# mmwillet/TTS.cpp

Measured on AMD Instinct MI355X. Metric: audio-seconds/sec (Parler-TTS-Mini fp16, greedy decode + DAC to 44.1 kHz PCM), higher is better.
Workload: dtype f16

## Files before the change

tts.cpp_amd/csrc/parler_kernels.h:

```cpp
#pragma once
#include <hip/hip_runtime.h>
#include <stdint.h>
#include <type_traits>

#include "wave_ops.h"

struct EmbedArgs {
    const void *tab;
    int         tab_f16;
    int64_t     tab_stride;
    int         n_tabs;
    const uint32_t *ids;
    const float *pos_embed;
    const uint32_t *row_pos;
    float      *x;
    int         H;
};

static __global__ void embed_rows_kernel(EmbedArgs a) {
    const int r = blockIdx.x;
    const uint32_t pos = a.row_pos[r];
    uint32_t id[16];
#pragma unroll
    for (int i = 0; i < 16; i++) id[i] = a.ids[r * a.n_tabs + min(i, a.n_tabs - 1)];
// ... 445 lines not shown
__global__ void gemv_valu_kernel(GemmArgs a, int EPI, int act_f16_src) {
    const int lane = threadIdx.x & 63, w = threadIdx.x >> 6;
    const int n = blockIdx.x * (blockDim.x >> 6) + w;
    if (n >= a.N) return;
    for (int r = 0; r < a.R; r++) {
        float acc = 0.0f;
        for (int k = lane; k < a.K; k += 64) {
            float wv, xv;
            if (WT == 1) wv = (float) ((const _Float16 *) a.W)[(int64_t) n * a.K + k];
            else         wv = ((const float *) a.W)[(int64_t) n * a.K + k];
            if (act_f16_src) xv = (float) ((const _Float16 *) a.A)[(int64_t) r * a.lda + k];
            else {
                xv = ((const float *) a.A)[(int64_t) r * a.lda + k];
                if (WT == 1) xv = (float) (_Float16) xv;
            }
            acc += wv * xv;
        }
        acc = wave_sum(acc);
        if (lane == 0) {
            if (EPI == EPI_STORE) a.out[(int64_t) r * a.ldo + n] = acc;
            else if (EPI == EPI_RESID) a.out[(int64_t) r * a.ldo + n] += acc;
            else if (EPI == EPI_GELU) {
                const float gl = gelu_apply(acc, a.gelu_mode);
                if (a.out16) a.out16[(int64_t) r * a.ldo + n] = (_Float16) gl;
                else a.out[(int64_t) r * a.ldo + n] = gl;
            } else {
                const int which = n / a.H, c = n - which * a.H;
                if (which == 0) a.q[(int64_t) r * a.H + c] = acc;
                else {
                    const int64_t off = (int64_t) a.row_seq[r] * a.seq_stride + (int64_t) a.row_pos[r] * a.H + c;
                    void *base = which == 1 ? a.kc : a.vc;
                    if (a.kv_f16) ((_Float16 *) base)[off] = (_Float16) acc;
                    else ((float *) base)[off] = acc;
                }
            }
        }
    }
}

__device__ __forceinline__ unsigned quant4_q8(float4v y, float &d_out);
template <int NI, int NP>
__device__ __forceinline__ void ln_row_regs(float *xr, int H, int lane, const float *lw, const float *lb, float *yr32, _Float16 *yr16,
                                            const float *pr, int n_parts, int64_t slab_stride, int8_t *yq = nullptr, float *ydT = nullptr, int ldr = 0) {
    float4v v[NI], w4[NI], b4[NI];
    float4v p[NP > 0 ? NP : 1][NI];
#pragma unroll
    for (int i = 0; i < NI; i++) {
        const int k = min(i * 256 + lane * 4, H - 4);
        v[i] = *(const float4v *) (xr + k);
#pragma unroll
        for (int sp = 0; sp < NP; sp++) p[sp][i] = *(const float4v *) (pr + sp * slab_stride + k);
        w4[i] = *(const float4v *) (lw + k);
        b4[i] = *(const float4v *) (lb + k);
    }
    if (NP != 0) {
#pragma unroll
        for (int i = 0; i < NI; i++) {
            const int k = i * 256 + lane * 4;
            if (k < H) {
                if (NP > 0) {
#pragma unroll
                    for (int sp = 0; sp < NP; sp++) v[i] += p[sp][i];
                } else {
                    for (int sp = 0; sp < n_parts; sp++) v[i] += *(const float4v *) (pr + sp * slab_stride + k);
                }
                *(float4v *) (xr + k) = v[i];
            }
        }
    }
    float s = 0.0f;
#pragma unroll
    for (int i = 0; i < NI; i++)
        if (i * 256 + lane * 4 < H) s += (v[i][0] + v[i][1]) + (v[i][2] + v[i][3]);
    const float mean = wave_sum(s) / (float) H;
    float s2 = 0.0f;
#pragma unroll
    for (int i = 0; i < NI; i++)
        if (i * 256 + lane * 4 < H) {
#pragma unroll
            for (int e = 0; e < 4; e++) { const float d = v[i][e] - mean; s2 += d * d; }
        }
    const float rstd = 1.0f / sqrtf(wave_sum(s2) / (float) H + LN_EPS);
#pragma unroll
    for (int i = 0; i < NI; i++) {
        const int k = i * 256 + lane * 4;
        if (k < H) {
            float4v y;
#pragma unroll
            for (int e = 0; e < 4; e++) y[e] = (v[i][e] - mean) * rstd * w4[i][e] + b4[i][e];
            if (yr32) *(float4v *) (yr32 + k) = y;
            if (yr16) {
                half4 h;
#pragma unroll
                for (int e = 0; e < 4; e++) h[e] = (_Float16) y[e];
                *(half4 *) (yr16 + k) = h;
            }
            if (yq) {
                float dd;
                const unsigned qq = quant4_q8(y, dd);
                *(unsigned *) (yq + k) = qq;
                if ((lane & 7) == 0) ydT[(int64_t) (k >> 5) * ldr] = dd;
            }
        }
    }
}

template <int NI, int NP>
__global__ __launch_bounds__(256) void ln_rows_t_kernel(float *x, int H, const float *lw, const float *lb, float *y32, _Float16 *y16, int R, const float *parts, int n_parts,
                                                        int64_t slab_stride) {
    const int lane = threadIdx.x & 63;
    const int r = blockIdx.x * (blockDim.x >> 6) + (threadIdx.x >> 6);
    if (r >= R) return;
    const float *pr = parts ? parts + (int64_t) r * H : nullptr;
    ln_row_regs<NI, NP>(x + (int64_t) r * H, H, lane, lw, lb, y32 ? y32 + (int64_t) r * H : nullptr, y16 ? y16 + (int64_t) r * H : nullptr, pr, parts ? n_parts : 0, slab_stride);
}

template <int NI, int NP>
__global__ __launch_bounds__(256) void ln_rows_q8t_kernel(float *x, int H, const float *lw, const float *lb, int8_t *q, float *dT, int ldr, int R, const float *parts, int n_parts,
                                                          int64_t slab_stride) {
    const int lane = threadIdx.x & 63;
    const int r = blockIdx.x * (blockDim.x >> 6) + (threadIdx.x >> 6);
    if (r >= R) return;
    const float *pr = parts ? parts + (int64_t) r * H : nullptr;
    ln_row_regs<NI, NP>(x + (int64_t) r * H, H, lane, lw, lb, (float *) nullptr, (_Float16 *) nullptr, pr, parts ? n_parts : 0, slab_stride, q + (int64_t) r * H, dT + r, ldr);
}

static __global__ __launch_bounds__(256) void ln_rows_kernel(float *x, int H, const float *lw, const float *lb, float *y32,
                                                      _Float16 *y16, int R, const float *parts, int n_parts, int64_t slab_stride) {
    const int lane = threadIdx.x & 63;
    const int r = blockIdx.x * (blockDim.x >> 6) + (threadIdx.x >> 6);
    if (r >= R) return;
    float *xr = x + (int64_t) r * H;
    if (parts)
        for (int k = lane; k < H; k += 64) {
            float v = xr[k];
            for (int sp = 0; sp < n_parts; sp++) v += parts[sp * slab_stride + (int64_t) r * H + k];
            xr[k] = v;
        }
    float s = 0.0f;
    for (int k = lane; k < H; k += 64) s += xr[k];
    const float mean = wave_sum(s) / (float) H;
    float s2 = 0.0f;
    for (int k = lane; k < H; k += 64) { const float d = xr[k] - mean; s2 += d * d; }
    const float rstd = 1.0f / sqrtf(wave_sum(s2) / (float) H + LN_EPS);
    for (int k = lane; k < H; k += 64) {
        const float y = (xr[k] - mean) * rstd * lw[k] + lb[k];
        if (y32) y32[(int64_t) r * H + k] = y;
        if (y16) y16[(int64_t) r * H + k] = (_Float16) y;
    }
}

struct AttnArgs {
    const float *q;
    const void *kc, *vc;
    int kv_f16;
    int64_t seq_stride;
    const uint32_t *row_seq, *row_pos;
    int T_fixed;
    int H, n_heads;
    float scale;
    float *out;
    _Float16 *out16;
    float *part;
    int max_T;
    uint32_t *counters;
    long long *stamps;
    int8_t *out_q;
    float *out_dT;
    int ldr;
};

__device__ __forceinline__ float4v load_kv4(const void *base, int kv_f16, int64_t off) {
    if (kv_f16) {
        const half4 h = *(const half4 *) ((const _Float16 *) base + off);
        return (float4v){(float) h[0], (float) h[1], (float) h[2], (float) h[3]};
    }
    return *(const float4v *) ((const float *) base + off);
}

template <bool KVF16>
__device__ __forceinline__ void attn_key_pass(const AttnArgs &a, int64_t hb, float4v q4, int tbeg, int t1, int step, int NKG, float &m, float &l, float4v &acc) {
    for (int t = tbeg; t < t1; t += step) {
        float4v k4[4], v4[4];
#pragma unroll
        for (int u = 0; u < 4; u++) {
            const int64_t off = hb + (int64_t) min(t + u * NKG, t1 - 1) * a.H;
            if (KVF16) {
                const half4 hk = *(const half4 *) ((const _Float16 *) a.kc + off), hv = *(const half4 *) ((const _Float16 *) a.vc + off);
                k4[u] = (float4v){(float) hk[0], (float) hk[1], (float) hk[2], (float) hk[3]};
                v4[u] = (float4v){(float) hv[0], (float) hv[1], (float) hv[2], (float) hv[3]};
            } else {
                k4[u] = *(const float4v *) ((const float *) a.kc + off);
                v4[u] = *(const float4v *) ((const float *) a.vc + off);
            }
        }
#pragma unroll
        for (int u = 0; u < 4; u++) {
            if (t + u * NKG < t1) {
                float d = q4[0] * k4[u][0] + q4[1] * k4[u][1] + q4[2] * k4[u][2] + q4[3] * k4[u][3];
                d = row16_sum(d);
                d *= a.scale;
                const float mn = fmaxf(m, d);
                const float f = expf(m - mn);
                const float p = expf(d - mn);
                l = l * f + p;
#pragma unroll
                for (int e = 0; e < 4; e++) acc[e] = acc[e] * f + p * v4[u][e];
                m = mn;
            }
        }
    }
}

static __global__ __launch_bounds__(1024) void attn_kernel(AttnArgs a) {
    extern __shared__ __attribute__((aligned(16))) char smem[];
    const int NKG = blockDim.x >> 4;
    float *red = (float *) smem;
    const int h = blockIdx.x, r = blockIdx.y, z = blockIdx.z, nz = gridDim.z;
    const int tid = threadIdx.x, kg = tid >> 4, cl = tid & 15, c4 = cl * 4;
    B1_STAMP(a.stamps, 0);
    const int T = a.row_pos ? (int) a.row_pos[r] + 1 : a.T_fixed;
    const int64_t sb = a.row_seq ? (int64_t) a.row_seq[r] * a.seq_stride : 0;
    const int chunk = (T + nz - 1) / nz;
    const int t0 = z * chunk, t1 = min(T, t0 + chunk);
    const int64_t hb = sb + h * 64 + c4;
    const float4v q4 = *(const float4v *) (a.q + (int64_t) r * a.H + h * 64 + c4);
    const int step = NKG * 4;

    float m = -INFINITY, l = 0.0f;
    float4v acc = {0.f, 0.f, 0.f, 0.f};
    if (a.kv_f16) attn_key_pass<true>(a, hb, q4, t0 + kg, t1, step, NKG, m, l, acc);
    else attn_key_pass<false>(a, hb, q4, t0 + kg, t1, step, NKG, m, l, acc);
    if (a.stamps != nullptr) { asm volatile("" :: "v"(acc[0])); B1_STAMP(a.stamps, 1); }
    if (cl == 0) red[NKG * 64 + kg] = m;
    __syncthreads();
    float mx = -INFINITY;
    for (int i = 0; i < NKG; i++) mx = fmaxf(mx, red[NKG * 64 + i]);
    const float f = (m == -INFINITY) ? 0.0f : expf(m - mx);
#pragma unroll
    for (int e = 0; e < 4; e++) acc[e] *= f;
    *(float4v *) (red + kg * 64 + c4) = acc;
    if (cl == 0) red[NKG * 65 + kg] = l * f;
    __syncthreads();
    if (tid < 64) {
        float o = 0.0f, s = 0.0f;
        for (int i = 0; i < NKG; i++) { o += red[i * 64 + tid]; s += red[NKG * 65 + i]; }
        if (nz == 1) {
            const float res = o / s;
            if (a.out16) a.out16[(int64_t) r * a.H + h * 64 + tid] = (_Float16) res;
            else a.out[(int64_t) r * a.H + h * 64 + tid] = res;
        } else {
            float *p = a.part + (((int64_t) r * a.n_heads + h) * nz + z) * ATT_PS;
            if (a.counters) {
                if (tid == 0) {
                    __hip_atomic_store(p, mx, __ATOMIC_RELAXED, __HIP_MEMORY_SCOPE_AGENT);
                    __hip_atomic_store(p + 1, s, __ATOMIC_RELAXED, __HIP_MEMORY_SCOPE_AGENT);
                }
                __hip_atomic_store(p + ATT_PO + tid, o, __ATOMIC_RELAXED, __HIP_MEMORY_SCOPE_AGENT);
            } else {
                if (tid == 0) { p[0] = mx; p[1] = s; }
                p[ATT_PO + tid] = o;
            }
        }
    }
    B1_STAMP(a.stamps, 2);
    if (nz == 1 || !a.counters) return;
    uint32_t *s_last = (uint32_t *) (red + NKG * 66);
    __syncthreads();
    if (tid == 0) {
        const uint32_t prev = __hip_atomic_fetch_add(a.counters + r * a.n_heads + h, 1u, __ATOMIC_ACQ_REL, __HIP_MEMORY_SCOPE_AGENT);
        *s_last = prev == (uint32_t) nz - 1 ? 1u : 0u;
    }
    __syncthreads();
    if (!*s_last || tid >= 64) return;
    const float *p = a.part + ((int64_t) r * a.n_heads + h) * nz * ATT_PS;
    float mm[16], ss[16], oo[16];
#pragma unroll
    for (int i = 0; i < 16; i++) {
        if (i < nz) {
            mm[i] = __hip_atomic_load(p + i * ATT_PS, __ATOMIC_RELAXED, __HIP_MEMORY_SCOPE_AGENT);
            ss[i] = __hip_atomic_load(p + i * ATT_PS + 1, __ATOMIC_RELAXED, __HIP_MEMORY_SCOPE_AGENT);
            oo[i] = __hip_atomic_load(p + i * ATT_PS + ATT_PO + tid, __ATOMIC_RELAXED, __HIP_MEMORY_SCOPE_AGENT);
        }
    }
    float gmx = -INFINITY;
#pragma unroll
    for (int i = 0; i < 16; i++) if (i < nz) gmx = fmaxf(gmx, mm[i]);
    float ot = 0.0f, st = 0.0f;
#pragma unroll
    for (int i = 0; i < 16; i++) {
        if (i < nz && mm[i] != -INFINITY) {
            const float f2 = expf(mm[i] - gmx);
            ot += f2 * oo[i];
            st += f2 * ss[i];
        }
    }
    const float res = ot / st;
    if (a.out16) a.out16[(int64_t) r * a.H + h * 64 + tid] = (_Float16) res;
    else a.out[(int64_t) r * a.H + h * 64 + tid] = res;
    if (tid == 0) __hip_atomic_store(a.counters + r * a.n_heads + h, 0u, __ATOMIC_RELAXED, __HIP_MEMORY_SCOPE_AGENT);
    if (a.stamps != nullptr && tid == 0 && (h == 0 || h == (int) gridDim.x - 1) && r == 0) a.stamps[(h ? 8 : 0) + 3] = (long long) __builtin_amdgcn_s_memrealtime();
}

template <bool KVF16, int U>
__device__ __forceinline__ void attn_row_pass(const AttnArgs &a, int64_t hb, float4v q4, int t0, int t1, float &m, float &l, float4v &acc) {
    for (int t = t0; t < t1; t += U) {
        float4v k4[U], v4[U];
#pragma unroll
        for (int u = 0; u < U; u++) {
            const int64_t off = hb + (int64_t) min(t + u, t1 - 1) * a.H;
            if (KVF16) {
                const half4 hk = __builtin_nontemporal_load((const half4 *) ((const _Float16 *) a.kc + off)), hv = __builtin_nontemporal_load((const half4 *) ((const _Float16 *) a.vc + off));
                k4[u] = (float4v){(float) hk[0], (float) hk[1], (float) hk[2], (float) hk[3]};
                v4[u] = (float4v){(float) hv[0], (float) hv[1], (float) hv[2], (float) hv[3]};
            } else {
                k4[u] = __builtin_nontemporal_load((const float4v *) ((const float *) a.kc + off));
                v4[u] = __builtin_nontemporal_load((const float4v *) ((const float *) a.vc + off));
            }
        }
#pragma unroll
        for (int u = 0; u < U; u++) {
            if (t + u < t1) {
                float d = q4[0] * k4[u][0] + q4[1] * k4[u][1] + q4[2] * k4[u][2] + q4[3] * k4[u][3];
                d = row16_sum(d);
                d *= a.scale;
                const float mn = fmaxf(m, d);
                const float f = expf(m - mn);
                const float p = expf(d - mn);
                l = l * f + p;
#pragma unroll
                for (int e = 0; e < 4; e++) acc[e] = acc[e] * f + p * v4[u][e];
                m = mn;
            }
        }
    }
}
template <int U>
__global__ __launch_bounds__(1024) void attn_rows_kernel(AttnArgs a) {
    const int r = blockIdx.x, z = blockIdx.y, nz = gridDim.y, tid = threadIdx.x;
    const int h = tid >> 4, cl = tid & 15;
    const int T = (int) a.row_pos[r] + 1;
    const int64_t sb = (int64_t) a.row_seq[r] * a.seq_stride;
    const int chunk = (T + nz - 1) / nz;
    const int t0 = z * chunk, t1 = min(T, t0 + chunk);
    const int64_t hb = sb + tid * 4;
    const float4v q4 = *(const float4v *) (a.q + (int64_t) r * a.H + tid * 4);
    float m = -INFINITY, l = 0.0f;
    float4v acc = {0.f, 0.f, 0.f, 0.f};
    if (t0 < t1) {
        if (a.kv_f16) attn_row_pass<true, U>(a, hb, q4, t0, t1, m, l, acc);
        else attn_row_pass<false, U>(a, hb, q4, t0, t1, m, l, acc);
    }
    if (nz == 1) {
        const float inv = 1.0f / l;
        if (a.out16) {
            half4 o;
#pragma unroll
            for (int e = 0; e < 4; e++) o[e] = (_Float16) (acc[e] * inv);
            *(half4 *) (a.out16 + (int64_t) r * a.H + tid * 4) = o;
        } else {
            float4v o;
#pragma unroll
            for (int e = 0; e < 4; e++) o[e] = acc[e] * inv;
            if (a.out_q) {
                float dd;
                const unsigned qq = quant4_q8(o, dd);
                *(unsigned *) (a.out_q + (int64_t) r * a.H + tid * 4) = qq;
                if ((tid & 7) == 0) a.out_dT[(int64_t) (tid >> 3) * a.ldr + r] = dd;
            } else {
                *(float4v *) (a.out + (int64_t) r * a.H + tid * 4) = o;
            }
        }
    } else {
        float *p = a.part + (((int64_t) r * a.n_heads + h) * nz + z) * ATT_PS;
        if (cl == 0) { p[0] = m; p[1] = l; }
        *(float4v *) (p + ATT_PO + cl * 4) = acc;
    }
}

template <int TN>
__device__ __forceinline__ void attn_short_body(const AttnArgs &a, int r, int h, int lane, int T) {
    const int64_t hb = h * 64 + lane;
    const float qv = a.q[(int64_t) r * a.H + hb];
    float kv[TN], vv[TN], sc[TN];
    const float *kc = (const float *) a.kc, *vc = (const float *) a.vc;
#pragma unroll
    for (int t = 0; t < TN; t++) {
        const int64_t off = hb + (int64_t) min(t, T - 1) * a.H;
        kv[t] = kc[off];
        vv[t] = vc[off];
    }
    float m = -INFINITY;
#pragma unroll
    for (int t = 0; t < TN; t++)
        if (t < T) { sc[t] = wave_sum(qv * kv[t]) * a.scale; m = fmaxf(m, sc[t]); }
    float l = 0.0f, o = 0.0f;
#pragma unroll
    for (int t = 0; t < TN; t++)
        if (t < T) { const float p = expf(sc[t] - m); l += p; o += p * vv[t]; }
    const float res = o / l;
    if (a.out16) a.out16[(int64_t) r * a.H + hb] = (_Float16) res;
    else a.out[(int64_t) r * a.H + hb] = res;
}
static __global__ __launch_bounds__(256) void attn_short_kernel(AttnArgs a) {
    const int lane = threadIdx.x & 63;
    const int h = blockIdx.x * (blockDim.x >> 6) + (threadIdx.x >> 6), r = blockIdx.y;
    if (h >= a.n_heads) return;
    B1_STAMP(a.stamps, 0);
    const int T = a.T_fixed;
    if (T <= 8) attn_short_body<8>(a, r, h, lane, T);
    else if (T <= 16) attn_short_body<16>(a, r, h, lane, T);
    else attn_short_body<32>(a, r, h, lane, T);
    B1_STAMP(a.stamps, 3);
}


static __global__ void attn_combine_kernel(const float *part, int nz, int H, int n_heads, float *out, _Float16 *out16, int8_t *out_q = nullptr, float *out_dT = nullptr, int ldr = 0) {
    const int h = blockIdx.x, r = blockIdx.y, c = threadIdx.x;
    const float *p = part + ((int64_t) r * n_heads + h) * nz * ATT_PS;
    float m[16], s[16], o[16];
#pragma unroll
    for (int z = 0; z < 16; z++) {
        if (z < nz) { m[z] = p[z * ATT_PS]; s[z] = p[z * ATT_PS + 1]; o[z] = p[z * ATT_PS + ATT_PO + c]; }
    }
    float mx = -INFINITY;
#pragma unroll
    for (int z = 0; z < 16; z++) if (z < nz) mx = fmaxf(mx, m[z]);
    float oo = 0.0f, ss = 0.0f;
#pragma unroll
    for (int z = 0; z < 16; z++) {
        if (z < nz && m[z] != -INFINITY) {
            const float f = expf(m[z] - mx);
            oo += f * o[z];
            ss += f * s[z];
        }
    }
    const float res = oo / ss;
    if (out_q) {
        const float amax = lanes32_max(fabsf(res));
        const float dd = amax / 127.0f;
        const float id = dd ? 1.0f / dd : 0.0f;
        out_q[(int64_t) r * H + h * 64 + c] = (int8_t) roundf(res * id);
        if ((c & 31) == 0) out_dT[(int64_t) (h * 2 + (c >> 5)) * ldr + r] = (float) (_Float16) dd;
    } else if (out16) out16[(int64_t) r * H + h * 64 + c] = (_Float16) res;
    else out[(int64_t) r * H + h * 64 + c] = res;
}

static __global__ void argmax_kernel(const float *logits, int V, uint32_t *tokens) {
    __shared__ float bv[4];
    __shared__ uint32_t bi[4];
    const int idx = blockIdx.x;
    const float *lg = logits + (int64_t) idx * V;
    float best = -INFINITY;
    uint32_t besti = 0;
    for (int i = threadIdx.x; i < V; i += blockDim.x) {
        const float v = lg[i];
        if (v > best) { best = v; besti = (uint32_t) i; }
    }
#pragma unroll
    for (int o = 32; o > 0; o >>= 1) {
        const float ov = __shfl_xor(best, o);
        const uint32_t oi = __shfl_xor(besti, o);
        if (ov > best || (ov == best && oi < besti)) { best = ov; besti = oi; }
    }
    const int w = threadIdx.x >> 6;
    if ((threadIdx.x & 63) == 0) { bv[w] = best; bi[w] = besti; }
    __syncthreads();
    if (threadIdx.x == 0) {
        for (int i = 1; i < (int) (blockDim.x >> 6); i++)
            if (bv[i] > best || (bv[i] == best && bi[i] < besti)) { best = bv[i]; besti = bi[i]; }
        tokens[idx] = besti;
    }
}

#define SMP_VMAX 2048
struct SampleArgs {
    const float *logits;
    int V, n_out, R;
    uint32_t top_k;
    float top_p, temperature;
    const float *uniforms;
    const uint32_t *row_step;
    uint32_t *out;
    const double *pen_table;
    int pen_len;
    int32_t *last_ids;
    uint32_t *rep_counts;
    const uint32_t *orig;
    int R_total;
};

__device__ __forceinline__ unsigned long long smp_key(float v, int i) {
    unsigned u = __float_as_uint(v == 0.0f ? 0.0f : v);
    u = (u & 0x80000000u) ? ~u : (u | 0x80000000u);
    return ((unsigned long long) (~u) << 32) | (unsigned) i;
}

__device__ __forceinline__ void smp_rank_select(const float *val, int V, int k, unsigned short *picks, unsigned long long *keys) {
    int P = 1;
    while (P < V) P <<= 1;
    for (int i = threadIdx.x; i < P; i += blockDim.x) keys[i] = i < V ? smp_key(val[i], i) : ~0ull;
    __syncthreads();
    for (int size = 2; size <= P; size <<= 1) {
        for (int stride = size >> 1; stride > 0; stride >>= 1) {
            for (int t = threadIdx.x; t < (P >> 1); t += blockDim.x) {
                const int lo = ((t / stride) * (stride << 1)) + (t % stride), hi = lo + stride;
                const bool up = ((lo & size) == 0);
                const unsigned long long a = keys[lo], b = keys[hi];
                if ((a > b) == up) { keys[lo] = b; keys[hi] = a; }
            }
            __syncthreads();
        }
    }
    for (int j = threadIdx.x; j < k; j += blockDim.x) picks[j] = (unsigned short) (keys[j] & 0xFFFFu);
}

static __global__ __launch_bounds__(256) void sample_kernel(SampleArgs a) {
    __shared__ float val[SMP_VMAX];
    __shared__ float tmp[SMP_VMAX];
    __shared__ unsigned short picks[SMP_VMAX];
    __shared__ unsigned long long keys[SMP_VMAX];
    __shared__ float bv[4];
    __shared__ uint32_t bi[4];
    __shared__ float s_top, s_total, s_mhp;
    __shared__ int s_n;
    const int h = blockIdx.x, r = blockIdx.y, tid = threadIdx.x, V = a.V;
    const float *row = a.logits + ((int64_t) r * a.n_out + h) * V;
    const bool temp = a.temperature != 1.0f;
    const bool use_topk = a.top_k > 0 && a.top_k < (uint32_t) V;
    const bool use_topp = a.top_p < 1.0f;

    const int ro = a.orig ? (int) a.orig[r] : r;
    const int last = a.pen_table ? a.last_ids[ro * a.n_out + h] : -1;
    float pen_v = 0.0f;
    if (last >= 0 && last < V) {
        const uint32_t cnt = a.rep_counts[ro * a.n_out + h];
        pen_v = (float) ((double) row[last] / a.pen_table[cnt < (uint32_t) a.pen_len ? cnt : (uint32_t) a.pen_len - 1]);
    }
    float best = -INFINITY;
    uint32_t besti = 0;
    for (int i = tid; i < V; i += 256) {
        const float v = i == last ? pen_v : row[i];
        val[i] = v;
        if (v > best) { best = v; besti = (uint32_t) i; }
    }
#pragma unroll
    for (int o = 32; o > 0; o >>= 1) {
        const float ov = __shfl_xor(best, o);
        const uint32_t oi = __shfl_xor(besti, o);
        if (ov > best || (ov == best && oi < besti)) { best = ov; besti = oi; }
    }
    if ((tid & 63) == 0) { bv[tid >> 6] = best; bi[tid >> 6] = besti; }
    __syncthreads();
    if (tid == 0) {
        for (int i = 1; i < 4; i++)
            if (bv[i] > best || (bv[i] == best && bi[i] < besti)) { best = bv[i]; besti = bi[i]; }
        float top = val[besti];
        if (temp) top /= a.temperature;
        s_top = top;
    }
    __syncthreads();
    const float top = s_top;
    int n = V;
    bool nucleus = false;

    if (use_topp) {
        for (int i = tid; i < V; i += 256) {
            float v = val[i];
            if (temp) v /= a.temperature;
            tmp[i] = expf(v - top);
        }
        __syncthreads();
        if (tid == 0) {
            float total = 0.0f;
            for (int i = 0; i < V; i++) total += tmp[i];
            s_total = total;
        }
        __syncthreads();
        for (int i = tid; i < V; i += 256) val[i] = tmp[i] / s_total;
        __syncthreads();
    }
    if (use_topk) {
        smp_rank_select(val, V, (int) a.top_k, picks, keys);
        n = (int) a.top_k;
        nucleus = true;
        __syncthreads();
    }
    if (!use_topp) {
        for (int j = tid; j < n; j += 256) {
            float v = val[nucleus ? picks[j] : j];
            if (temp) v /= a.temperature;
            tmp[j] = expf(v - top);
        }
        __syncthreads();
        if (tid == 0) {
            float total = 0.0f;
            for (int j = 0; j < n; j++) total += tmp[j];
            s_total = total;
        }
        __syncthreads();
        for (int j = tid; j < n; j += 256) val[nucleus ? picks[j] : j] = tmp[j] / s_total;
        __syncthreads();
    } else {
        if (!nucleus) {
            smp_rank_select(val, V, V, picks, keys);
            nucleus = true;
            __syncthreads();
        }
        if (tid == 0) {
            float mass = 0.0f;
            int keep = -1;
            for (int j = 0; j < n; j++) {
                mass += val[picks[j]];
                if (mass >= a.top_p) { keep = j + 1; break; }
            }
            s_mhp = fminf(mass, a.top_p);
            s_n = keep > 0 ? keep : n;
        }
        __syncthreads();
        n = s_n;
    }
    if (tid == 0) {
        const uint32_t call = a.row_step ? a.row_step[r] - 1 : 0;
        const float u = a.uniforms[((int64_t) call * (a.orig ? a.R_total : a.R) + ro) * a.n_out + h];
        const float target = use_topp ? u * s_mhp : u;
        float cum = 0.0f;
        int chosen = n ? (nucleus ? (int) picks[n - 1] : n - 1) : 0;
        for (int j = 0; j < n; j++) {
            const int i = nucleus ? (int) picks[j] : j;
            cum += val[i];
            if (target <= cum || j + 1 >= n) { chosen = i; break; }
        }
        a.out[r * a.n_out + h] = (uint32_t) chosen;
        if (a.pen_table) {
            uint32_t cnt = a.rep_counts[ro * a.n_out + h];
            if (last != chosen) cnt = 0;
            a.last_ids[ro * a.n_out + h] = chosen;
            a.rep_counts[ro * a.n_out + h] = cnt + 1;
        }
    }
}

struct FeedArgs {
    const uint32_t *tokens;
    uint32_t *ids;
    uint32_t *row_pos;
    uint32_t *row_step;
    uint8_t  *eos_seen;
    uint32_t *steps_done;
    uint32_t *tokens_out;
    int R, n_out;
    uint32_t bos, eos;
    uint32_t max_pos;
    const uint32_t *orig;
// ... 242 lines not shown
```

Before: 1016.

## Double-buffer K/V loads in row attention and pin waves per EU

```diff
diff --git a/profiles/attn_rows_bench.hip b/profiles/attn_rows_bench.hip
--- /dev/null
+++ b/profiles/attn_rows_bench.hip
@@ -0,0 +1,339 @@
+#include <hip/hip_runtime.h>
+#include <cstdio>
+#include <cstdlib>
+#include <cstring>
+#include <cmath>
+#include <vector>
+#include <algorithm>
+#include "../tts.cpp_amd/csrc/parler_kernels.h"
+#define CK(x) do { hipError_t e = (x); if (e != hipSuccess) { printf("HIP error %s line %d\n", hipGetErrorString(e), __LINE__); exit(1); } } while (0)
+
+typedef AttnArgs Args;
+
+__global__ void fill_kernel(float *p, size_t n, uint32_t seed, float amp) {
+    for (size_t i = (size_t) blockIdx.x * blockDim.x + threadIdx.x; i < n; i += (size_t) gridDim.x * blockDim.x) {
+        uint32_t x = (uint32_t) i * 2654435761u ^ (uint32_t) (i >> 32) ^ seed;
+        x ^= x >> 16; x *= 0x7feb352du; x ^= x >> 15; x *= 0x846ca68bu; x ^= x >> 16;
+        p[i] = ((float) (x & 0xffffff) / 8388608.0f - 1.0f) * amp;
+    }
+}
+
+template <bool CLAMP>
+__global__ __launch_bounds__(1024) void probe_kernel(Args a) {
+    const int r = blockIdx.x, tid = threadIdx.x;
+    const int T = (int) a.row_pos[r] + 1;
+    const int64_t hb = (int64_t) a.row_seq[r] * a.seq_stride + tid * 4;
+    float4v acc = {0.f, 0.f, 0.f, 0.f};
+    for (int t = 0; t < T; t += 8) {
+        float4v k4[8], v4[8];
+#pragma unroll
+        for (int u = 0; u < 8; u++) {
+            if (CLAMP || t + u < T) {
+                const int64_t off = hb + (int64_t) min(t + u, T - 1) * a.H;
+                k4[u] = __builtin_nontemporal_load((const float4v *) ((const float *) a.kc + off));
+                v4[u] = __builtin_nontemporal_load((const float4v *) ((const float *) a.vc + off));
+            } else {
+                k4[u] = v4[u] = (float4v){0.f, 0.f, 0.f, 0.f};
+            }
+        }
+#pragma unroll
+        for (int u = 0; u < 8; u++) {
+            typedef int int4v __attribute__((ext_vector_type(4)));
+            const int4v x = __builtin_bit_cast(int4v, k4[u]) ^ __builtin_bit_cast(int4v, v4[u]) ^ __builtin_bit_cast(int4v, acc);
+            acc = __builtin_bit_cast(float4v, x);
+        }
+    }
+    if (__builtin_bit_cast(unsigned, acc[0]) == 0x12345678u && __builtin_bit_cast(unsigned, acc[1]) == 0x9abcdef0u) a.out[tid] = acc[2] + acc[3];
+}
+
+template <bool KVF16, int U>
+__device__ __forceinline__ void parent_row_pass(const AttnArgs &a, int64_t hb, float4v q4, int t0, int t1, float &m, float &l, float4v &acc) {
+    for (int t = t0; t < t1; t += U) {
+        float4v k4[U], v4[U];
+#pragma unroll
+        for (int u = 0; u < U; u++) {
+            const int64_t off = hb + (int64_t) min(t + u, t1 - 1) * a.H;
+            if (KVF16) {
+                const half4 hk = __builtin_nontemporal_load((const half4 *) ((const _Float16 *) a.kc + off)), hv = __builtin_nontemporal_load((const half4 *) ((const _Float16 *) a.vc + off));
+                k4[u] = (float4v){(float) hk[0], (float) hk[1], (float) hk[2], (float) hk[3]};
+                v4[u] = (float4v){(float) hv[0], (float) hv[1], (float) hv[2], (float) hv[3]};
+            } else {
+                k4[u] = __builtin_nontemporal_load((const float4v *) ((const float *) a.kc + off));
+                v4[u] = __builtin_nontemporal_load((const float4v *) ((const float *) a.vc + off));
+            }
+        }
+#pragma unroll
+        for (int u = 0; u < U; u++) {
+            if (t + u < t1) {
+                float d = q4[0] * k4[u][0] + q4[1] * k4[u][1] + q4[2] * k4[u][2] + q4[3] * k4[u][3];
+                d = row16_sum(d);
+                d *= a.scale;
+                const float mn = fmaxf(m, d);
+                const float f = expf(m - mn);
+                const float p = expf(d - mn);
+                l = l * f + p;
+#pragma unroll
+                for (int e = 0; e < 4; e++) acc[e] = acc[e] * f + p * v4[u][e];
+                m = mn;
+            }
+        }
+    }
+}
+template <int U>
+__global__ __launch_bounds__(1024) void parent_rows_kernel(AttnArgs a) {
+    const int r = blockIdx.x, z = blockIdx.y, nz = gridDim.y, tid = threadIdx.x;
+    const int h = tid >> 4, cl = tid & 15;
+    const int T = (int) a.row_pos[r] + 1;
+    const int64_t sb = (int64_t) a.row_seq[r] * a.seq_stride;
+    const int chunk = (T + nz - 1) / nz;
+    const int t0 = z * chunk, t1 = min(T, t0 + chunk);
+    const int64_t hb = sb + tid * 4;
+    const float4v q4 = *(const float4v *) (a.q + (int64_t) r * a.H + tid * 4);
+    float m = -INFINITY, l = 0.0f;
+    float4v acc = {0.f, 0.f, 0.f, 0.f};
+    if (t0 < t1) {
+        if (a.kv_f16) parent_row_pass<true, U>(a, hb, q4, t0, t1, m, l, acc);
+        else parent_row_pass<false, U>(a, hb, q4, t0, t1, m, l, acc);
+    }
+    if (nz == 1) {
+        const float inv = 1.0f / l;
+        if (a.out16) {
+            half4 o;
+#pragma unroll
+            for (int e = 0; e < 4; e++) o[e] = (_Float16) (acc[e] * inv);
+            *(half4 *) (a.out16 + (int64_t) r * a.H + tid * 4) = o;
+        } else {
+            float4v o;
+#pragma unroll
+            for (int e = 0; e < 4; e++) o[e] = acc[e] * inv;
+            if (a.out_q) {
+                float dd;
+                const unsigned qq = quant4_q8(o, dd);
+                *(unsigned *) (a.out_q + (int64_t) r * a.H + tid * 4) = qq;
+                if ((tid & 7) == 0) a.out_dT[(int64_t) (tid >> 3) * a.ldr + r] = dd;
+            } else {
+                *(float4v *) (a.out + (int64_t) r * a.H + tid * 4) = o;
+            }
+        }
+    } else {
+        float *p = a.part + (((int64_t) r * a.n_heads + h) * nz + z) * ATT_PS;
+        if (cl == 0) { p[0] = m; p[1] = l; }
+        *(float4v *) (p + ATT_PO + cl * 4) = acc;
+    }
+}
+
+template <int U> using KV = AttnGroup<false, U>;
+template <int U>
+__device__ __forceinline__ void issue(KV<U> &b, const float *rk, const float *rv, int H, int t, int tl, unsigned lo) {
+    attn_issue_group<false, U>(b, (const char *) rk, (const char *) rv, (int64_t) H * 4, t, tl, lo);
+}
+template <int U, bool SKIPF>
+__device__ __forceinline__ void fold(const KV<U> &b, float4v q4, float scale, int t, int t1, float &m, float &l, float4v &acc) {
+    if (!SKIPF) { attn_fold_group<false, U, false>(b, q4, scale, t, t1, m, l, acc); return; }
+#pragma unroll
+    for (int u = 0; u < U; u++) {
+        if (t + u < t1) {
+#pragma clang fp contract(off)
+            const float4v k = b.k[u], v = b.v[u];
+            float d = q4[0] * k[0] + q4[1] * k[1];
+            d = q4[2] * k[2] + d;
+            d = q4[3] * k[3] + d;
+            d = row16_sum(d);
+            const float mn = fmaxf(m, d * scale);
+            const float p = expf(__builtin_fmaf(scale, d, -mn));
+            float f = 1.0f;
+            if (__builtin_amdgcn_ballot_w64(mn != m) != 0) f = mn == m ? 1.0f : expf(m - mn);
+            l = __builtin_fmaf(l, f, p);
+            acc[0] = __builtin_fmaf(v[0], p, acc[0] * f);
+            acc[1] = __builtin_fmaf(v[1], p, acc[1] * f);
+            acc[2] = v[2] * p + acc[2] * f;
+            acc[3] = v[3] * p + acc[3] * f;
+            m = mn;
+        }
+    }
+}
+
+template <int U, bool PIPE, int THREADS, int MINB, bool PERSIST, bool SKIPF>
+__global__ __launch_bounds__(THREADS, MINB) __attribute__((amdgpu_waves_per_eu(THREADS * MINB / 256, THREADS * MINB / 256))) void var_kernel(Args a) {
+    const int tid = threadIdx.x;
+    const unsigned lo = (unsigned) (blockIdx.y * THREADS + tid) * 16u;
+    const int G = gridDim.x;
+    int r = blockIdx.x;
+    if (!PERSIST) {
+        const int T = (int) a.row_pos[r] + 1;
+        const int64_t sb = (int64_t) a.row_seq[r] * a.seq_stride;
+        const float *rk = (const float *) a.kc + sb, *rv = (const float *) a.vc + sb;
+        const float4v q4 = *(const float4v *) ((const char *) (a.q + (int64_t) r * a.H) + lo);
+        float m = -INFINITY, l = 0.0f;
+        float4v acc = {0.f, 0.f, 0.f, 0.f};
+        if (PIPE) {
+            KV<U> A, B;
+            issue<U>(A, rk, rv, a.H, 0, T - 1, lo);
+            for (int t = 0; t < T; t += 2 * U) {
+                issue<U>(B, rk, rv, a.H, t + U, T - 1, lo);
+                fold<U, SKIPF>(A, q4, a.scale, t, T, m, l, acc);
+                if (t + U >= T) break;
+                issue<U>(A, rk, rv, a.H, t + 2 * U, T - 1, lo);
+                fold<U, SKIPF>(B, q4, a.scale, t + U, T, m, l, acc);
+            }
+        } else {
+            for (int t = 0; t < T; t += U) {
+                KV<U> A;
+                issue<U>(A, rk, rv, a.H, t, T - 1, lo);
+                fold<U, SKIPF>(A, q4, a.scale, t, T, m, l, acc);
+            }
+        }
+        const float inv = 1.0f / l;
+        float4v o;
+#pragma unroll
+        for (int e = 0; e < 4; e++) o[e] = acc[e] * inv;
+        *(float4v *) ((char *) (a.out + (int64_t) r * a.H) + lo) = o;
+    } else {
+        int pr = r, pt = 0, pT = (int) a.row_pos[r] + 1;
+        int64_t psb = (int64_t) a.row_seq[r] * a.seq_stride;
+        float4v pq = *(const float4v *) ((const char *) (a.q + (int64_t) r * a.H) + lo);
+        int cr = r, ct = 0, cT = pT;
+        float4v q4 = pq;
+        float m = -INFINITY, l = 0.0f;
+        float4v acc = {0.f, 0.f, 0.f, 0.f};
+        KV<U> A, B;
+        issue<U>(A, (const float *) a.kc + psb, (const float *) a.vc + psb, a.H, 0, pT - 1, lo);
+#define ADVANCE_AND_ISSUE(BUF) \
+        pt += U; \
+        if (pt >= pT && pr + G < a.T_fixed ) { \
+            pr += G; pt = 0; pT = (int) a.row_pos[pr] + 1; psb = (int64_t) a.row_seq[pr] * a.seq_stride; \
+            pq = *(const float4v *) ((const char *) (a.q + (int64_t) pr * a.H) + lo); \
+        } \
+        issue<U>(BUF, (const float *) a.kc + psb, (const float *) a.vc + psb, a.H, pt, pT - 1, lo);
+#define FOLD_AND_STEP(BUF) \
+        fold<U, SKIPF>(BUF, q4, a.scale, ct, cT, m, l, acc); \
+        ct += U; \
+        if (ct >= cT) { \
+            const float inv = 1.0f / l; \
+            float4v o; \
+            for (int e = 0; e < 4; e++) o[e] = acc[e] * inv; \
+            *(float4v *) ((char *) (a.out + (int64_t) cr * a.H) + lo) = o; \
+            cr += G; \
+            if (cr >= a.T_fixed ) break; \
+            ct = 0; cT = pT; q4 = pq; m = -INFINITY; l = 0.0f; acc = (float4v){0.f, 0.f, 0.f, 0.f}; \
+        }
+        for (;;) {
+            ADVANCE_AND_ISSUE(B)
+            FOLD_AND_STEP(A)
+            ADVANCE_AND_ISSUE(A)
+            FOLD_AND_STEP(B)
+        }
+#undef ADVANCE_AND_ISSUE
+#undef FOLD_AND_STEP
+    }
+}
+
+struct Bench {
+    Args a;
+    std::vector<float> h_ref, h_out;
+    size_t n_out;
+    int R;
+    double bytes;
+    int T;
+};
+
+template <typename F>
+static float time_launch(F launch, int reps) {
+    hipEvent_t e0, e1; CK(hipEventCreate(&e0)); CK(hipEventCreate(&e1));
+    launch(); launch();
+    CK(hipDeviceSynchronize());
+    std::vector<float> ms(reps);
+    for (int i = 0; i < reps; i++) {
+        CK(hipEventRecord(e0));
+        launch();
+        CK(hipEventRecord(e1)); CK(hipEventSynchronize(e1));
+        CK(hipEventElapsedTime(&ms[i], e0, e1));
+    }
+    CK(hipGetLastError());
+    std::sort(ms.begin(), ms.end());
+    CK(hipEventDestroy(e0)); CK(hipEventDestroy(e1));
+    return ms[reps / 2];
+}
+
+static void report(const Bench &b, const char *name, float ms, const char *extra) {
+    printf("T %4d  %-34s %8.1f us  %5.2f TB/s  %s\n", b.T, name, ms * 1e3, b.bytes / ms / 1e9, extra);
+    fflush(stdout);
+}
+
+template <int U, bool PIPE, int THREADS, int MINB, bool PERSIST, bool SKIPF>
+static void run_var(Bench &b, const char *name, int persist_grid = 0) {
+    auto kern = var_kernel<U, PIPE, THREADS, MINB, PERSIST, SKIPF>;
+    int per_cu = 0;
+    CK(hipOccupancyMaxActiveBlocksPerMultiprocessor(&per_cu, kern, THREADS, 0));
+    const dim3 grid(PERSIST ? persist_grid : b.R, 1024 / THREADS);
+    CK(hipMemset(b.a.out, 0xff, b.n_out * 4));
+    const float ms = time_launch([&] { hipLaunchKernelGGL(kern, grid, dim3(THREADS), 0, 0, b.a); }, 21);
+    CK(hipMemcpy(b.h_out.data(), b.a.out, b.n_out * 4, hipMemcpyDeviceToHost));
+    const bool same = memcmp(b.h_out.data(), b.h_ref.data(), b.n_out * 4) == 0;
+    char extra[96];
+    snprintf(extra, sizeof extra, "%d workgroups/CU  %s", per_cu, same ? "bit-equal to parent" : "DIFFERS FROM parent");
+    report(b, name, ms, extra);
+}
+
+int main(int argc, char **argv) {
+    std::vector<int> Ts;
+    for (int i = 1; i < argc; i++) Ts.push_back(atoi(argv[i]));
+    if (Ts.empty()) Ts = {137, 272};
+    const int R = 1024, H = 1024, NPOS = 288;
+    hipDeviceProp_t prop; CK(hipGetDeviceProperties(&prop, 0));
+    const int cus = prop.multiProcessorCount;
+    printf("%s, %d CUs\n", prop.name, cus);
+    float *q, *kc, *vc, *out; uint32_t *row_seq, *row_pos;
+    const size_t ncache = (size_t) R * NPOS * H;
+    CK(hipMalloc(&q, (size_t) R * H * 4)); CK(hipMalloc(&kc, ncache * 4)); CK(hipMalloc(&vc, ncache * 4)); CK(hipMalloc(&out, (size_t) R * H * 4));
+    CK(hipMalloc(&row_seq, R * 4)); CK(hipMalloc(&row_pos, R * 4));
+    hipLaunchKernelGGL(fill_kernel, dim3(4096), dim3(256), 0, 0, q, (size_t) R * H, 1u, 1.0f);
+    hipLaunchKernelGGL(fill_kernel, dim3(4096), dim3(256), 0, 0, kc, ncache, 2u, 2.0f);
+    hipLaunchKernelGGL(fill_kernel, dim3(4096), dim3(256), 0, 0, vc, ncache, 3u, 1.0f);
+    CK(hipDeviceSynchronize());
+    std::vector<uint32_t> seq(R), pos(R);
+    for (int r = 0; r < R; r++) seq[r] = r;
+    CK(hipMemcpy(row_seq, seq.data(), R * 4, hipMemcpyHostToDevice));
+    for (int T : Ts) {
+        if (T < 1 || T > NPOS) { printf("T %d outside 1..%d\n", T, NPOS); continue; }
+        for (int r = 0; r < R; r++) pos[r] = T - 1;
+        CK(hipMemcpy(row_pos, pos.data(), R * 4, hipMemcpyHostToDevice));
+        Bench b;
+        memset(&b.a, 0, sizeof b.a);
+        b.a.q = q; b.a.kc = kc; b.a.vc = vc; b.a.seq_stride = (int64_t) NPOS * H; b.a.row_seq = row_seq; b.a.row_pos = row_pos;
+        b.a.T_fixed = R; b.a.H = H; b.a.n_heads = H / 64; b.a.scale = 0.125f; b.a.out = out; b.R = R;
+        b.n_out = (size_t) R * H; b.T = T;
+        b.bytes = 2.0 * T * H * 4 * R;
+        b.h_ref.resize(b.n_out); b.h_out.resize(b.n_out);
+        report(b, "probe (read only, clamped tail)", time_launch([&] { hipLaunchKernelGGL(probe_kernel<true>, dim3(R), dim3(1024), 0, 0, b.a); }, 21), "");
+        report(b, "probe_x (tail requests dropped)", time_launch([&] { hipLaunchKernelGGL(probe_kernel<false>, dim3(R), dim3(1024), 0, 0, b.a); }, 21), "");
+        report(b, "parent attn_rows_kernel<8>", time_launch([&] { hipLaunchKernelGGL(parent_rows_kernel<8>, dim3(R), dim3(1024), 0, 0, b.a); }, 21), "");
+        CK(hipMemcpy(b.h_ref.data(), out, b.n_out * 4, hipMemcpyDeviceToHost));
+        for (int which = 0; which < 2; which++) {
+            CK(hipMemset(out, 0xff, b.n_out * 4));
+            const float ms = which ? time_launch([&] { hipLaunchKernelGGL(attn_rows_kernel<16>, dim3(R), dim3(1024), 0, 0, b.a); }, 21)
+                                   : time_launch([&] { hipLaunchKernelGGL(attn_rows_kernel<8>, dim3(R), dim3(1024), 0, 0, b.a); }, 21);
+            CK(hipMemcpy(b.h_out.data(), out, b.n_out * 4, hipMemcpyDeviceToHost));
+            report(b, which ? "parler_kernels.h attn_rows_kernel<16>" : "parler_kernels.h attn_rows_kernel<8>", ms,
+                   memcmp(b.h_out.data(), b.h_ref.data(), b.n_out * 4) == 0 ? "bit-equal to parent" : "DIFFERS FROM parent");
+        }
+        run_var<8, false, 1024, 1, false, false>(b, "U8 uniform row pointers");
+        run_var<8, false, 1024, 1, false, true>(b, "U8 + skipf");
+        run_var<4, false, 1024, 2, false, false>(b, "U4, 2 wg/CU asked");
+        run_var<4, false, 1024, 2, false, true>(b, "U4, 2 wg/CU asked + skipf");
+        run_var<8, true, 1024, 1, false, false>(b, "U8 pipe");
+        run_var<8, true, 1024, 1, false, true>(b, "U8 pipe + skipf");
+        run_var<4, true, 1024, 1, false, false>(b, "U4 pipe");
+        run_var<4, true, 1024, 1, false, true>(b, "U4 pipe + skipf");
+        run_var<8, false, 512, 2, false, false>(b, "half rows U8, 2 wg/CU");
+        run_var<8, true, 512, 2, false, false>(b, "half rows U8 pipe, 2 wg/CU");
+        run_var<8, true, 512, 2, false, true>(b, "half rows U8 pipe + skipf");
+        run_var<4, true, 512, 4, false, false>(b, "half rows U4 pipe, 4 wg/CU asked");
+        run_var<4, true, 512, 4, false, true>(b, "half rows U4 pipe + skipf, 4 asked");
+        run_var<8, true, 1024, 1, true, false>(b, "persistent U8 pipe, G = CUs", cus);
+        run_var<8, true, 1024, 1, true, true>(b, "persistent U8 pipe + skipf", cus);
+        run_var<4, true, 1024, 2, true, false>(b, "persistent U4 pipe, G = 2 CUs", 2 * cus);
+        run_var<4, true, 1024, 2, true, true>(b, "persistent U4 pipe + skipf, 2 CUs", 2 * cus);
+    }
+    return 0;
+}
diff --git a/tts.cpp_amd/csrc/parler_kernels.h b/tts.cpp_amd/csrc/parler_kernels.h
--- a/tts.cpp_amd/csrc/parler_kernels.h
+++ b/tts.cpp_amd/csrc/parler_kernels.h
@@ -771,54 +771,87 @@
     if (a.stamps != nullptr && tid == 0 && (h == 0 || h == (int) gridDim.x - 1) && r == 0) a.stamps[(h ? 8 : 0) + 3] = (long long) __builtin_amdgcn_s_memrealtime();
 }
 
+template <bool KVF16> struct AttnRaw { typedef float4v type; };
+template <> struct AttnRaw<true> { typedef half4 type; };
+template <bool KVF16, int U> struct AttnGroup { typename AttnRaw<KVF16>::type k[U], v[U]; };
+
+__device__ __forceinline__ float4v attn_widen(float4v x) { return x; }
+__device__ __forceinline__ float4v attn_widen(half4 x) { return (float4v){(float) x[0], (float) x[1], (float) x[2], (float) x[3]}; }
+
 template <bool KVF16, int U>
-__device__ __forceinline__ void attn_row_pass(const AttnArgs &a, int64_t hb, float4v q4, int t0, int t1, float &m, float &l, float4v &acc) {
-    for (int t = t0; t < t1; t += U) {
-        float4v k4[U], v4[U];
-#pragma unroll
-        for (int u = 0; u < U; u++) {
-            const int64_t off = hb + (int64_t) min(t + u, t1 - 1) * a.H;
-            if (KVF16) {
-                const half4 hk = __builtin_nontemporal_load((const half4 *) ((const _Float16 *) a.kc + off)), hv = __builtin_nontemporal_load((const half4 *) ((const _Float16 *) a.vc + off));
-                k4[u] = (float4v){(float) hk[0], (float) hk[1], (float) hk[2], (float) hk[3]};
-                v4[u] = (float4v){(float) hv[0], (float) hv[1], (float) hv[2], (float) hv[3]};
-            } else {
-                k4[u] = __builtin_nontemporal_load((const float4v *) ((const float *) a.kc + off));
-                v4[u] = __builtin_nontemporal_load((const float4v *) ((const float *) a.vc + off));
-            }
-        }
-#pragma unroll
-        for (int u = 0; u < U; u++) {
-            if (t + u < t1) {
-                float d = q4[0] * k4[u][0] + q4[1] * k4[u][1] + q4[2] * k4[u][2] + q4[3] * k4[u][3];
-                d = row16_sum(d);
-                d *= a.scale;
-                const float mn = fmaxf(m, d);
-                const float f = expf(m - mn);
-                const float p = expf(d - mn);
-                l = l * f + p;
-#pragma unroll
-                for (int e = 0; e < 4; e++) acc[e] = acc[e] * f + p * v4[u][e];
-                m = mn;
-            }
-        }
+__device__ __forceinline__ void attn_issue_group(AttnGroup<KVF16, U> &g, const char *rk, const char *rv, int64_t key_bytes, int t, int tl, unsigned lo) {
+    typedef typename AttnRaw<KVF16>::type raw;
+#pragma unroll
+    for (int u = 0; u < U; u++) {
+        const int64_t ro = (int64_t) min(t + u, tl) * key_bytes;
+        g.k[u] = __builtin_nontemporal_load((const raw *) (rk + ro + lo));
+        g.v[u] = __builtin_nontemporal_load((const raw *) (rv + ro + lo));
+    }
+}
+
+__device__ __forceinline__ void attn_fold_key(float4v q4, float4v k, float4v v, float scale, float &m, float &l, float4v &acc) {
+#pragma clang fp contract(off)
+    float d = q4[0] * k[0] + q4[1] * k[1];
+    d = q4[2] * k[2] + d;
+    d = q4[3] * k[3] + d;
+    d = row16_sum(d);
+    const float mn = fmaxf(m, d * scale);
+    const float f = expf(m - mn);
+    const float p = expf(__builtin_fmaf(scale, d, -mn));
+    l = __builtin_fmaf(l, f, p);
+    acc[0] = __builtin_fmaf(v[0], p, acc[0] * f);
+    acc[1] = __builtin_fmaf(v[1], p, acc[1] * f);
+    acc[2] = v[2] * p + acc[2] * f;
+    acc[3] = v[3] * p + acc[3] * f;
+    m = mn;
+}
+
+template <bool KVF16, int U, bool FULL>
+__device__ __forceinline__ void attn_fold_group(const AttnGroup<KVF16, U> &g, float4v q4, float scale, int t, int t1, float &m, float &l, float4v &acc) {
+#pragma unroll
+    for (int u = 0; u < U; u++)
+        if (FULL || t + u < t1) attn_fold_key(q4, attn_widen(g.k[u]), attn_widen(g.v[u]), scale, m, l, acc);
+}
+
+template <bool KVF16, int U>
+__device__ __forceinline__ void attn_row_pass(const AttnArgs &a, int64_t sb, unsigned lo4, float4v q4, int t0, int t1, float &m, float &l, float4v &acc) {
+    constexpr int ESZ = KVF16 ? 2 : 4, G = U / 2;
+    const char *rk = (const char *) a.kc + sb * ESZ, *rv = (const char *) a.vc + sb * ESZ;
+    const int64_t key_bytes = (int64_t) a.H * ESZ;
+    const unsigned lo = lo4 * ESZ;
+    AttnGroup<KVF16, G> ga, gb;
+    attn_issue_group<KVF16, G>(ga, rk, rv, key_bytes, t0, t1 - 1, lo);
+    int t = t0;
+    for (; t + U <= t1; t += U) {
+        attn_issue_group<KVF16, G>(gb, rk, rv, key_bytes, t + G, t1 - 1, lo);
+        __builtin_amdgcn_sched_barrier(0);
+        attn_fold_group<KVF16, G, true>(ga, q4, a.scale, t, t1, m, l, acc);
+        __builtin_amdgcn_sched_barrier(0);
+        attn_issue_group<KVF16, G>(ga, rk, rv, key_bytes, t + U, t1 - 1, lo);
+        __builtin_amdgcn_sched_barrier(0);
+        attn_fold_group<KVF16, G, true>(gb, q4, a.scale, t + G, t1, m, l, acc);
+        __builtin_amdgcn_sched_barrier(0);
+    }
+    if (t < t1) {
+        if (t + G < t1) attn_issue_group<KVF16, G>(gb, rk, rv, key_bytes, t + G, t1 - 1, lo);
+        attn_fold_group<KVF16, G, false>(ga, q4, a.scale, t, t1, m, l, acc);
+        if (t + G < t1) attn_fold_group<KVF16, G, false>(gb, q4, a.scale, t + G, t1, m, l, acc);
     }
 }
 template <int U>
-__global__ __launch_bounds__(1024) void attn_rows_kernel(AttnArgs a) {
+__global__ __launch_bounds__(1024) __attribute__((amdgpu_waves_per_eu(4, 4))) void attn_rows_kernel(AttnArgs a) {
     const int r = blockIdx.x, z = blockIdx.y, nz = gridDim.y, tid = threadIdx.x;
     const int h = tid >> 4, cl = tid & 15;
     const int T = (int) a.row_pos[r] + 1;
     const int64_t sb = (int64_t) a.row_seq[r] * a.seq_stride;
     const int chunk = (T + nz - 1) / nz;
     const int t0 = z * chunk, t1 = min(T, t0 + chunk);
-    const int64_t hb = sb + tid * 4;
     const float4v q4 = *(const float4v *) (a.q + (int64_t) r * a.H + tid * 4);
     float m = -INFINITY, l = 0.0f;
     float4v acc = {0.f, 0.f, 0.f, 0.f};
     if (t0 < t1) {
-        if (a.kv_f16) attn_row_pass<true, U>(a, hb, q4, t0, t1, m, l, acc);
-        else attn_row_pass<false, U>(a, hb, q4, t0, t1, m, l, acc);
+        if (a.kv_f16) attn_row_pass<true, U>(a, sb, (unsigned) tid * 4u, q4, t0, t1, m, l, acc);
+        else attn_row_pass<false, U>(a, sb, (unsigned) tid * 4u, q4, t0, t1, m, l, acc);
     }
     if (nz == 1) {
         const float inv = 1.0f / l;
```

Result: slower. 1005 (-1.1%).
